# E3SM-Project/PAM

Measured on AMD Instinct MI355X. Metric: cell-updates/sec (AWFL dycore step), higher is better.
Workload: dtype f64; 1 GPU; AWFL supercell idealized, nens=1024/GPU, 32x32x60 L60, NT=1, fp64; scaling=weak, nens_total=1024, nens_per_gpu=1024, nx=32, ny=32, nz=60, num_tracers=1, parallelism=nens-shard x1, ranks_seen=1, limiter_input=0, fct_rows_flagged_last_stage=0, fct_rows=983040, lanes=member+xsweep

## Files before the change

### pam_amd/csrc/awfl_device.h

```cpp
#pragma once
#include <math.h>
#include <stdint.h>
#include <string.h>
#include <type_traits>
#include "awfl_constants.h"

#if defined(__HIPCC__)
#define PAMA_D __device__ __forceinline__
#else
#define PAMA_D inline
#endif

namespace pama {

constexpr int HS = 3;
constexpr int MAXT = 50;
constexpr int FLUX_THREADS = 256;
constexpr int FLUX_WAVES = FLUX_THREADS / 64;
#ifndef PAMA_FLUX_NF
#define PAMA_FLUX_NF 2
#endif
constexpr int FLUX_NF = PAMA_FLUX_NF;
constexpr int FLUX_MAX_SPAN = 64;
constexpr int VZ_STRIDE = 31;
// ... 1119 lines not shown
      const bool limited = (m != 1.0);
      if (limited) {
        rows.flags[(long long)t * fct_rows_per_tracer(P) + fct_row(P, k, j, i, e)] = rows.seq;
        rows.any[e >> 6] = rows.seq;
      }
      if (rows.sparse_store) store = wave_any(limited);
    }
    if (store) mult[(long long)t * P.ncell + idx] = m;
  }
}

PAMA_D double limited_flux(double F, double ml, double mh, bool seam) {
  if (F > 0.0) return mul_rn(F, ml);
  if (F < 0.0) return seam ? F : mul_rn(F, mh);
  return F;
}



struct NearFlags { bool c, im1, ip1, jm1, jp1, km1, kp1; };
PAMA_D bool any_of(const NearFlags &g) { return g.c | g.im1 | g.ip1 | g.jm1 | g.jp1 | g.km1 | g.kp1; }
PAMA_D NearFlags fct_near_flags(const Params &P, const FctRows &rows, int t, int k, int j, int i, int e) {
  const long long lstride = (long long)((P.nens + 63) >> 6) * P.nx;
  const int *fl = rows.flags + (long long)t * fct_rows_per_tracer(P) + fct_row(P, k, j, i, e);
  const long long r_ip1 = (i == P.nx - 1) ? -(long long)(P.nx - 1) : 1, r_im1 = (i == 0) ? (long long)(P.nx - 1) : -1;
  const long long r_jp1 = ((j == P.ny - 1) ? -(long long)(P.ny - 1) : 1) * lstride, r_jm1 = ((j == 0) ? (long long)(P.ny - 1) : -1) * lstride;
  const long long r_kz = (long long)P.ny * lstride;
  const bool zl = (k > 0), zh = (k < P.nz - 1);
  const int sq = rows.seq;
  const int a0 = fl[0], a1 = fl[r_im1], a2 = fl[r_ip1], a3 = fl[r_jm1], a4 = fl[r_jp1], a5 = fl[zl ? -r_kz : 0], a6 = fl[zh ? r_kz : 0];
  NearFlags g;
  g.c = (a0 == sq); g.im1 = (a1 == sq); g.ip1 = (a2 == sq); g.jm1 = (a3 == sq); g.jp1 = (a4 == sq);
  g.km1 = zl & (a5 == sq); g.kp1 = zh & (a6 == sq);
  return g;
}
PAMA_D bool fct_flagged_near(const Params &P, const FctRows &rows, int t, int k, int j, int i, int e) {
  return any_of(fct_near_flags(P, rows, t, k, j, i, e));
}

template <int STAGE>
PAMA_D void tracer_new_value(const Params &P, int t, double f_x, double f_xp1, double f_y, double f_yp1, double f_z, double f_zp1,
                             double q_in, double q_0, double rho_in, double rho_0, double rdzk, double dt_dyn, double &v,
                             double &new_seed) {
  const double tend = flux_divergence(P, f_x, f_xp1, f_y, f_yp1, f_z, f_zp1, rdzk);
  const double m_in = mul_rn(q_in, rho_in);
  double m_0 = 0.0;
  if (STAGE > 1) m_0 = mul_rn(q_0, rho_0);
  v = rk_combine<STAGE>(m_0, m_in, dt_dyn, tend);
  if ((P.pos_mask >> t) & 1ull) v = fmax(0.0, v);
  new_seed = next_seed<STAGE>(m_0, m_in, v);
}

template <int STAGE>
PAMA_D void tracer_update_one(const Params &P, int t, const double *prim_in, const double *prim0, double *prim_out,
                              const double *__restrict__ fx, const double *__restrict__ fy, const double *__restrict__ fz,
                              const double *__restrict__ mult, const FctRows &rows, double *__restrict__ seed, double dt_dyn,
                              const CellId &c, double rho_in, double rho_0, double rrho, double rdzk, bool only_near_flagged) {
  const int k = c.k, j = c.j, i = c.i, e = c.e;
  const long long idx = c.idx;
  const long long c2 = (long long)j * P.sy + (long long)i * P.sx + e;
  const long long o = (long long)(k + HS) * P.sz + c2;
  const long long ip1 = idx + ((i == P.nx - 1) ? -(long long)(P.nx - 1) * P.sx : P.sx);
  const long long im1 = idx + ((i == 0) ? (long long)(P.nx - 1) * P.sx : -P.sx);
  const long long jp1 = idx + ((j == P.ny - 1) ? -(long long)(P.ny - 1) * P.sy : P.sy);
  const long long jm1 = idx + ((j == 0) ? (long long)(P.ny - 1) * P.sy : -P.sy);
  const double *tx = fx + (long long)(5 + t) * P.ncell, *ty = fy + (long long)(5 + t) * P.ncell;
  const double *tz = fz + (long long)(5 + t) * P.fz_fs;
  const double *mt = mult + (long long)t * P.ncell;
  if (only_near_flagged && rows.flags) {
    if (!wave_any_or_lane(fct_flagged_near(P, rows, t, k, j, i, e))) return;
  }
  const bool zlo = (k > 0), zhi = (k < P.nz - 1);
  double m_c = 1.0, m_im1 = 1.0, m_ip1 = 1.0, m_jm1 = 1.0, m_jp1 = 1.0, m_km1 = 1.0, m_kp1 = 1.0;
  const double Fx = tx[idx], Fxp1 = tx[ip1], Fz = tz[idx], Fzp1 = tz[idx + P.sz];
  const double Fy = P.sim2d ? 0.0 : ty[idx], Fyp1 = P.sim2d ? 0.0 : ty[jp1];
  const int pf = P_TR0 + t;
  const double q_in = prim_in[pf * P.prim_fs + o];
  const double q_0 = (STAGE > 1) ? prim0[pf * P.prim_fs + o] : 0.0;
  if (rows.flags) {
    const NearFlags g = fct_near_flags(P, rows, t, k, j, i, e);
    if (wave_any(any_of(g))) {
      const double l_c = mt[idx], l_im1 = mt[im1], l_ip1 = mt[ip1], l_jm1 = mt[jm1], l_jp1 = mt[jp1];
      const double l_km1 = mt[zlo ? idx - P.sz : idx], l_kp1 = mt[zhi ? idx + P.sz : idx];
      m_c = g.c ? l_c : 1.0; m_im1 = g.im1 ? l_im1 : 1.0; m_ip1 = g.ip1 ? l_ip1 : 1.0;
      m_jm1 = g.jm1 ? l_jm1 : 1.0; m_jp1 = g.jp1 ? l_jp1 : 1.0;
      m_km1 = g.km1 ? l_km1 : 1.0; m_kp1 = g.kp1 ? l_kp1 : 1.0;
    }
  } else {
    m_c = mt[idx]; m_im1 = mt[im1]; m_ip1 = mt[ip1];
    if (!P.sim2d) { m_jm1 = mt[jm1]; m_jp1 = mt[jp1]; }
    if (zlo) m_km1 = mt[idx - P.sz];
    if (zhi) m_kp1 = mt[idx + P.sz];
  }
  double f_x = limited_flux(Fx, m_im1, m_c, i == 0);
  double f_xp1 = limited_flux(Fxp1, m_c, m_ip1, i == P.nx - 1);
  double f_y = 0.0, f_yp1 = 0.0;
  if (!P.sim2d) {
    f_y = limited_flux(Fy, m_jm1, m_c, j == 0);
    f_yp1 = limited_flux(Fyp1, m_c, m_jp1, j == P.ny - 1);
  }
  const double f_z = limited_flux(Fz, m_km1, m_c, false);
  const double f_zp1 = limited_flux(Fzp1, m_c, m_kp1, false);
  double v, new_seed;
  tracer_new_value<STAGE>(P, t, f_x, f_xp1, f_y, f_yp1, f_z, f_zp1, q_in, q_0, rho_in, rho_0, rdzk, dt_dyn, v, new_seed);
  seed[(long long)t * P.ncell + idx] = new_seed;
  store_adv(P, prim_out, pf, k, c2, v * rrho, v * rrho);
}

template <int STAGE>
PAMA_D void tracer_update_part(const Params &P, const double *prim_in, const double *prim0, double *prim_out,
                               const double *__restrict__ fx, const double *__restrict__ fy, const double *__restrict__ fz,
                               const double *__restrict__ mult, const FctRows &rows, double *__restrict__ seed, double dt_dyn,
                               const CellId &c, double rho_in, double rho_0, double rrho, double rdzk) {
  for (int t = 0; t < P.nt; t++)
    tracer_update_one<STAGE>(P, t, prim_in, prim0, prim_out, fx, fy, fz, mult, rows, seed, dt_dyn, c, rho_in, rho_0, rrho, rdzk, false);
}

template <int STAGE>
PAMA_D void tracer_fixup_line_body(const Params &P, const double *prim_in, const double *prim0, double *prim_out,
                                   const double *__restrict__ fx, const double *__restrict__ fy, const double *__restrict__ fz,
                                   const double *__restrict__ mult, const FctRows &rows, double *__restrict__ seed, double dt_dyn,
                                   int t, int k, int j, int e) {
  {
    const int *ln = rows.lines + (long long)t * fct_lines_per_tracer(P);
    const int sq = rows.seq;
    const bool zl = (k > 0), zh = (k < P.nz - 1);
    const int jm = (j == 0) ? P.ny - 1 : j - 1, jp = (j == P.ny - 1) ? 0 : j + 1;
    const int a0 = ln[fct_line(P, k, j, e)], a1 = ln[fct_line(P, k, jm, e)], a2 = ln[fct_line(P, k, jp, e)];
    const int a3 = ln[fct_line(P, zl ? k - 1 : k, j, e)], a4 = ln[fct_line(P, zh ? k + 1 : k, j, e)];
    if (!wave_any_or_lane((a0 == sq) | (a1 == sq) | (a2 == sq) | (a3 == sq) | (a4 == sq))) return;
  }
  const double rdzk = fast_rcp(P.dz[(long long)k * P.nens + e]);
  for (int i = 0; i < P.nx; i++) {
    if (!wave_any_or_lane(fct_flagged_near(P, rows, t, k, j, i, e))) continue;
    CellId c;
    c.k = k; c.j = j; c.i = i; c.e = e;
    c.idx = (((long long)k * P.ny + j) * P.nx + i) * P.nens + e;
    const long long o = (long long)(k + HS) * P.sz + (long long)j * P.sy + (long long)i * P.sx + e;
    const double rho_new = prim_out[P_RHO * P.prim_fs + o];
    const double rho_in = prim_in[P_RHO * P.prim_fs + o];
    const double rho_0 = (STAGE > 1) ? prim0[P_RHO * P.prim_fs + o] : 0.0;
    tracer_update_one<STAGE>(P, t, prim_in, prim0, prim_out, fx, fy, fz, mult, rows, seed, dt_dyn, c, rho_in, rho_0,
                             fast_rcp(rho_new), rdzk, false);
  }
}

template <int STAGE>
PAMA_D void tracer_fixup_cell_body(const Params &P, const double *prim_in, const double *prim0, double *prim_out,
                                   const double *__restrict__ fx, const double *__restrict__ fy, const double *__restrict__ fz,
                                   const double *__restrict__ mult, const FctRows &rows, double *__restrict__ seed, double dt_dyn,
                                   int t, const CellId &c) {
  const int k = c.k, j = c.j, e = c.e;
  {
    const int *ln = rows.lines + (long long)t * fct_lines_per_tracer(P);
    const int sq = rows.seq;
    const bool zl = (k > 0), zh = (k < P.nz - 1);
    const int jm = (j == 0) ? P.ny - 1 : j - 1, jp = (j == P.ny - 1) ? 0 : j + 1;
    const int a0 = ln[fct_line(P, k, j, e)], a1 = ln[fct_line(P, k, jm, e)], a2 = ln[fct_line(P, k, jp, e)];
    const int a3 = ln[fct_line(P, zl ? k - 1 : k, j, e)], a4 = ln[fct_line(P, zh ? k + 1 : k, j, e)];
    if (!wave_any_or_lane((a0 == sq) | (a1 == sq) | (a2 == sq) | (a3 == sq) | (a4 == sq))) return;
  }
  if (!wave_any_or_lane(fct_flagged_near(P, rows, t, k, j, c.i, e))) return;
  const double rdzk = fast_rcp(P.dz[(long long)k * P.nens + e]);
  const long long o = (long long)(k + HS) * P.sz + (long long)j * P.sy + (long long)c.i * P.sx + e;
  const double rho_new = prim_out[P_RHO * P.prim_fs + o];
  const double rho_in = prim_in[P_RHO * P.prim_fs + o];
  const double rho_0 = (STAGE > 1) ? prim0[P_RHO * P.prim_fs + o] : 0.0;
  tracer_update_one<STAGE>(P, t, prim_in, prim0, prim_out, fx, fy, fz, mult, rows, seed, dt_dyn, c, rho_in, rho_0,
                           fast_rcp(rho_new), rdzk, false);
}

PAMA_D void pressure_tail_body(const Params &P, double *prim_out, const CellId &c) {
  const long long c2 = (long long)c.j * P.sy + (long long)c.i * P.sx + c.e;
  const long long o = (long long)(c.k + HS) * P.sz + c2;
  const bool boundary = (c.k == 0 || c.k == P.nz - 1);
  const double th = boundary ? prim_out[P_THETA * P.prim_fs + o] : 0.0;
  const double rho_theta = prim_out[P_PRES * P.prim_fs + o];
  const double rho_new = boundary ? prim_out[P_RHO * P.prim_fs + o] : 0.0;
  store_rho_pres<false>(P, prim_out, c.k, c2, c.e, rho_new, th, rho_theta, !P.grav_balance);
}

template <int STAGE>
PAMA_D void update_body(const Params &P, const double *prim_in, const double *prim0,
                        double *prim_out, const double *__restrict__ fx, const double *__restrict__ fy,
                        const double *__restrict__ fz, const double *__restrict__ mult, const FctRows &rows,
                        double *__restrict__ seed, double dt_dyn, const CellId &c) {
  const int k = c.k, j = c.j, i = c.i, e = c.e;
  const long long idx = c.idx;
  const long long c2 = (long long)j * P.sy + (long long)i * P.sx + e;
  const long long o = (long long)(k + HS) * P.sz + c2;
  const long long ke = (long long)k * P.nens + e;
  const double dzk = P.dz[ke];
  const double rdzk = fast_rcp(dzk);
  const long long ip1 = idx + ((i == P.nx - 1) ? -(long long)(P.nx - 1) * P.sx : P.sx);
  const long long im1 = idx + ((i == 0) ? (long long)(P.nx - 1) * P.sx : -P.sx);
  const long long jp1 = idx + ((j == P.ny - 1) ? -(long long)(P.ny - 1) * P.sy : P.sy);
  const long long jm1 = idx + ((j == 0) ? (long long)(P.ny - 1) * P.sy : -P.sy);
  const double rho_in = prim_in[P_RHO * P.prim_fs + o];
  const double rho_0 = (STAGE > 1) ? prim0[P_RHO * P.prim_fs + o] : 0.0;
  double qs[5];
#pragma unroll
  for (int l = 0; l < 5; l++) {
    const double *sx_ = fx + (long long)l * P.ncell, *sy_ = fy + (long long)l * P.ncell, *sz_ = fz + (long long)l * P.fz_fs;
    const double ylo = P.sim2d ? 0.0 : sy_[idx], yhi = P.sim2d ? 0.0 : sy_[jp1];
    double tend = (l == 0) ? flux_divergence(P, sx_[idx], sx_[ip1], ylo, yhi, sz_[idx], sz_[idx + P.sz], rdzk)
                           : flux_divergence_d(P, sx_[idx], sx_[ip1], ylo - yhi, sz_[idx] - sz_[idx + P.sz], rdzk);
    if (l == 3) tend = add_gravity(P, tend, rho_in, gravity_coef(P, ke));
    if (l == 2 && P.sim2d) tend = 0.0;
    const int pf = (l == 0) ? P_RHO : P_U + (l - 1);
    double m_in = prim_in[pf * P.prim_fs + o];
    if (l > 0) m_in = mul_rn(m_in, rho_in);
    double m_0 = 0.0;
    if (STAGE > 1) {
      m_0 = prim0[pf * P.prim_fs + o];
      if (l > 0) m_0 = mul_rn(m_0, rho_0);
    }
    qs[l] = rk_combine<STAGE>(m_0, m_in, dt_dyn, tend);
  }
  const double rrho = fast_rcp(qs[0]);
  const double th = qs[4] * rrho;
  tracer_update_part<STAGE>(P, prim_in, prim0, prim_out, fx, fy, fz, mult, rows, seed, dt_dyn, c, rho_in, rho_0, rrho, rdzk);
  store_rho_pres(P, prim_out, k, c2, e, qs[0], th, qs[4], !P.grav_balance);
// ... 170 lines not shown
          }
          const double f_z = limited_flux(zl[n], m_km1[n], mB[n], false);
          const double f_zp1 = limited_flux(zh[n], mB[n], m_kp1[n], false);
          double v, new_seed;
          tracer_new_value<STAGE>(P, tt[n], f_x, f_xp1, f_y, f_yp1, f_z, f_zp1, w[n][1], q_0[n], rho_in, rho_0, rdzk, dt_dyn, v, new_seed);
          uniw(seed + (long long)tt[n] * P.ncell + ix)[eu] = new_seed;
          store_adv_u(P, prim_out, P_TR0 + tt[n], k, cu0 + (long long)cc * P.sx, eu, v * rrho, v * rrho);
        }
      }
      F_prev[n] = F;
      prevR[n] = R[n];
      mA[n] = mB[n];
      mB[n] = m_new[n];
#pragma unroll
      for (int s = 0; s < 4; s++) w[n][s] = w[n][s + 1];
      w[n][4] = nq[n];
    }
  }
}

template <int STAGE, bool FOLD = false>
PAMA_D void flux_x_update_body(const Params &P, const double *__restrict__ prim_in, const double *__restrict__ prim0,
                               double *__restrict__ prim_out, double *__restrict__ fx, const double *__restrict__ fy,
                               const double *__restrict__ fz, double *__restrict__ seed, double *__restrict__ mult,
                               const FctRows &rows, int line, int e, int c0, int span, double dt_dyn, double dt_stage,
                               bool tracers_inline) {
  const unsigned eu = member_offset(e);
  const WenoConsts wc = weno_consts();
  const int nx = P.nx;
  const int c1 = (c0 + span < nx) ? c0 + span : nx;
  const int k = uni_int(line / P.ny), j = line - k * P.ny;
  const long long cu0 = (long long)j * P.sy;
  const long long pbase = (long long)(k + HS) * P.sz + cu0;
  const long long fbase = (long long)k * P.sz + cu0;
  const long long jp1 = (j == P.ny - 1) ? -(long long)(P.ny - 1) * P.sy : P.sy;
  const long long ke = (long long)k * P.nens + e;
  const double dzk = P.dz[ke];
  const double rdzk = fast_rcp(dzk);
  const double gcoef = gravity_coef(P, ke);
  const bool have_y = !P.sim2d;
  double ruf_close = 0.0;
  double *ruf_line = fx + fbase;
  auto cell_off = [&](int c) -> long long { return pbase + (long long)(c < 0 ? c + nx : (c >= nx ? c - nx : c)) * P.sx; };

  {
    constexpr int NQ = 4;
    const double *pr = prim_in + (long long)P_RHO * P.prim_fs;
    const double *pp = prim_in + (long long)P_PRES * P.prim_fs;
    const double *r0 = prim0 + (long long)P_RHO * P.prim_fs;
    double *out_rho = prim_out + (long long)P_RHO * P.prim_fs, *out_rt = prim_out + (long long)P_PRES * P.prim_fs;
    double wm[5], wp[5], wq[NQ][5], wt[5];
    const int tr = P.idWV;
    const double *pt = prim_in + (long long)(P_TR0 + tr) * P.prim_fs;
    double *flt = fx + (long long)(5 + tr) * P.ncell + fbase;
    const bool more_tracers = P.nt > 1;
    auto load_cell = [&](long long o, double &m, double &p, double (&qv)[NQ]) {
#pragma unroll
      for (int n = 0; n < NQ; n++) qv[n] = uni(prim_in + (long long)(P_U + n) * P.prim_fs + o)[eu];
      m = mul_rn(uni(pr + o)[eu], qv[0]);
      p = uni(pp + o)[eu];
    };
#pragma unroll
    for (int s = 0; s < 5; s++) {
      double qv[NQ];
      load_cell(cell_off(c0 - 3 + s), wm[s], wp[s], qv);
#pragma unroll
      for (int n = 0; n < NQ; n++) wq[n][s] = qv[n];
      wt[s] = uni(pt + cell_off(c0 - 3 + s))[eu];
    }
    double prevR_m, prevR_p, prevR_q[NQ], prevR_t;
    {
      double L;
      weno5_const(wm, wc, L, prevR_m);
      weno5_const(wp, wc, L, prevR_p);
      weno5_const(wt, wc, L, prevR_t);
#pragma unroll
      for (int n = 0; n < NQ; n++) {
        if (n == 1 && !have_y) { prevR_q[n] = 0.0; continue; }
        weno5_const(wq[n], wc, L, prevR_q[n]);
      }
      double nm, np_, nq[NQ];
      load_cell(cell_off(c0 + 2), nm, np_, nq);
      const double nt0 = uni(pt + cell_off(c0 + 2))[eu];
#pragma unroll
      for (int s = 0; s < 4; s++) {
        wm[s] = wm[s + 1]; wp[s] = wp[s + 1]; wt[s] = wt[s + 1];
#pragma unroll
        for (int n = 0; n < NQ; n++) wq[n][s] = wq[n][s + 1];
      }
      wm[4] = nm; wp[4] = np_; wt[4] = nt0;
#pragma unroll
      for (int n = 0; n < NQ; n++) wq[n][4] = nq[n];
    }
    double F_prev[1 + NQ], Ft_prev = 0.0;
#pragma unroll
    for (int l = 0; l <= NQ; l++) F_prev[l] = 0.0;
    struct CellIn { double rho_in, rho_0, q0[NQ], y0l, y0h, z0l, z0h, dy[1 + NQ], dz[1 + NQ], tyl, tyh, tzl, tzh, tseed, tq0; };
    const double *fyt = fy + (long long)(5 + tr) * P.ncell, *fzt = fz + (long long)(5 + tr) * P.fz_fs;
    const double *pt0 = prim0 + (long long)(P_TR0 + tr) * P.prim_fs;
    const double *sdt = seed + (long long)tr * P.ncell;
    auto load_in = [&](int cc, CellIn &ci) {
      const long long o = pbase + (long long)cc * P.sx, ix = fbase + (long long)cc * P.sx;
      ci.rho_in = uni(pr + o)[eu];
      ci.rho_0 = (STAGE > 1) ? uni(r0 + o)[eu] : 0.0;
#pragma unroll
      for (int n = 0; n < NQ; n++) ci.q0[n] = (STAGE > 1) ? uni(prim0 + (long long)(P_U + n) * P.prim_fs + o)[eu] : 0.0;
      ci.y0l = have_y ? uni(fy + ix)[eu] : 0.0;
// ... 7 lines not shown
      }
      ci.tyl = have_y ? uni(fyt + ix)[eu] : 0.0;
      ci.tyh = have_y ? uni(fyt + ix + jp1)[eu] : 0.0;
      ci.tzl = uni(fzt + ix)[eu];
      ci.tzh = uni(fzt + ix + P.sz)[eu];
      ci.tseed = uni(sdt + ix)[eu];
      ci.tq0 = (STAGE > 1) ? uni(pt0 + o)[eu] : 0.0;
    };
    auto finish = [&](int cc, const CellIn &ci, const double (&Flo)[1 + NQ], const double (&Fhi)[1 + NQ], double m_in_u,
                      double v_in, double w_in, double th_in, double Ft_lo, double Ft_hi, double qt_in) {
      const long long o = pbase + (long long)cc * P.sx;
      const double q0 = rk_combine<STAGE>(ci.rho_0, ci.rho_in, dt_dyn,
                                          flux_divergence(P, Flo[0], Fhi[0], ci.y0l, ci.y0h, ci.z0l, ci.z0h, rdzk));
      const double rrho = fast_rcp(q0);
      uniw(out_rho + o)[eu] = q0;
      const double q_in[NQ] = {0.0, v_in, w_in, th_in};
#pragma unroll
      for (int n = 0; n < NQ; n++) {
        const int l = 1 + n;
        double tend = FOLD ? flux_divergence_g(P, Flo[l], Fhi[l], ci.dz[l]) : flux_divergence_d(P, Flo[l], Fhi[l], ci.dy[l], ci.dz[l], rdzk);
        if (l == 3) tend = add_gravity(P, tend, ci.rho_in, gcoef);
        if (l == 2 && P.sim2d) tend = 0.0;
        const double m_in = (n == 0) ? m_in_u : mul_rn(q_in[n], ci.rho_in);
        const double m_0 = (STAGE > 1) ? mul_rn(ci.q0[n], ci.rho_0) : 0.0;
        const double v = rk_combine<STAGE>(m_0, m_in, dt_dyn, tend);
        store_adv_u(P, prim_out, P_U + n, k, cu0 + (long long)cc * P.sx, eu, v * rrho, (l == 3) ? 0.0 : v * rrho);
        if (l == 4) uniw(out_rt + o)[eu] = v;
      }
      finish_tracer_cell<STAGE>(P, tr, prim_out, seed, mult, rows, k, j, cc, e, eu, cu0 + (long long)cc * P.sx, fbase + (long long)cc * P.sx,
                                Ft_lo, Ft_hi, ci.tyl, ci.tyh, ci.tzl, ci.tzh, ci.tseed, qt_in, ci.tq0, ci.rho_in, ci.rho_0, rrho, dzk,
                                rdzk, dt_dyn, dt_stage);
    };
#pragma clang loop unroll(disable)
    for (int c = c0; c <= c1; c++) {
      double nm, np_, nq[NQ];
      load_cell(cell_off(c + 3), nm, np_, nq);
      const double nt0 = uni(pt + cell_off(c + 3))[eu];
      CellIn ci;
      load_in(c > c0 ? c - 1 : c0, ci);
      double Lm, Rm, Lp, Rp, Lq[NQ], Rq[NQ];
      weno5_const(wm, wc, Lm, Rm);
      weno5_const(wp, wc, Lp, Rp);
#pragma unroll
      for (int n = 0; n < NQ; n++) {
        if (n == 1 && !have_y) { Lq[n] = Rq[n] = 0.0; continue; }
        weno5_const(wq[n], wc, Lq[n], Rq[n]);
      }
      double Lt, Rt;
      weno5_const(wt, wc, Lt, Rt);
      double ruf, ppf, F[1 + NQ];
      acoustic_face(prevR_m, Lm, prevR_p, Lp, false, ruf, ppf);
      const bool up = ruf > 0.0;
      const double Ft = mul_rn(ruf, up ? prevR_t : Lt);
      if (c < c1) {
        if (more_tracers) uniw(ruf_line + (long long)c * P.sx)[eu] = ruf;
        uniw(flt + (long long)c * P.sx)[eu] = Ft;
      }
      ruf_close = ruf;
      F[0] = ruf;
      F[1] = fma(ruf, up ? prevR_q[0] : Lq[0], ppf);
#pragma unroll
      for (int n = 1; n < NQ; n++) F[1 + n] = mul_rn(ruf, up ? prevR_q[n] : Lq[n]);
      if (c > c0) finish(c - 1, ci, F_prev, F, wm[1], wq[1][1], wq[2][1], wq[3][1], Ft_prev, Ft, wt[1]);
#pragma unroll
      for (int l = 0; l <= NQ; l++) F_prev[l] = F[l];
      Ft_prev = Ft;
      prevR_m = Rm; prevR_p = Rp; prevR_t = Rt;
#pragma unroll
      for (int n = 0; n < NQ; n++) prevR_q[n] = Rq[n];
#pragma unroll
      for (int s = 0; s < 4; s++) {
        wm[s] = wm[s + 1]; wp[s] = wp[s + 1]; wt[s] = wt[s + 1];
#pragma unroll
        for (int n = 0; n < NQ; n++) wq[n][s] = wq[n][s + 1];
      }
      wm[4] = nm; wp[4] = np_; wt[4] = nt0;
#pragma unroll
      for (int n = 0; n < NQ; n++) wq[n][4] = nq[n];
    }
  }

  if (tracers_inline) {
    for (int i = 0; i < P.nt - 1; i += FLUX_NF) {
      const int fa[2] = {4 + further_tracer(P, i), 4 + further_tracer(P, i + 1)};
      if (i + 1 < P.nt - 1) x_tracer_sweep<2, STAGE, 1>(P, prim_in, prim0, prim_out, fx, fy, fz, seed, mult, rows, line, e, c0, span, fa, dt_dyn, dt_stage, true, ruf_close);
      else x_tracer_sweep<1, STAGE, 1>(P, prim_in, prim0, prim_out, fx, fy, fz, seed, mult, rows, line, e, c0, span, fa, dt_dyn, dt_stage, true, ruf_close);
    }
  }
}

struct XTileGeom {
  int W;
  int nmb;
  int tc;
  int halo;
  int ntl;
  int lpb;
};
PAMA_HD int xtile_rows(const XTileGeom &G) { return G.tc + 2 * G.halo; }
PAMA_HD int xtile_threads(const XTileGeom &G) { return G.W * xtile_rows(G) * G.lpb; }
PAMA_HD XTileGeom xtile_geometry(const Params &P, int w_req, int tc_req, int lpb_req, int ncu = 0) {
  XTileGeom G;
  G.W = (P.nens <= 64) ? P.nens : 64;
  if (P.nens < 64 && (long long)P.nx * P.nens > 512) {
    const int nmb = (int)(((long long)P.nx * P.nens + 511) / 512), w = (P.nens + nmb - 1) / nmb;
    if (w >= 16 && P.nx * w <= 1024) G.W = w;
    else if ((long long)P.nx * P.nens > 1024) {
      const int nmb2 = (int)(((long long)P.nx * P.nens + 1023) / 1024), w2 = (P.nens + nmb2 - 1) / nmb2;
      if (w2 >= 16 && P.nx * w2 <= 1024) G.W = w2;
    }
// ... 783 lines not shown
```

### pam_amd/csrc/awfl_kernels.hip

```cpp
#include <hip/hip_runtime.h>

#include <cmath>
#include <cstdio>
#include <cstring>
#include <atomic>
#include <map>
#include <mutex>
#include <string>
#include <vector>

#include "../../include/pam_amd_awfl.h"
#include "awfl_device.h"
#include "awfl_vertical.h"

using namespace pama;

struct EnsRange { int e0, ne; };
__device__ __forceinline__ long long to_global(long long t, int nens, EnsRange R) {
  const long long r = t / R.ne;
  return r * nens + R.e0 + (t - r * R.ne);
}

__device__ __forceinline__ bool flat_cell(const Params &P, int nlev, CellId &c) {
  const unsigned t = blockIdx.x * blockDim.x + threadIdx.x;
// ... 240 lines not shown
  if (t >= (unsigned)P.nx * (unsigned)R.ne) return;
  CellId c;
  const unsigned i = t / (unsigned)R.ne;
  c.j = by; c.i = (int)i; c.e = R.e0 + (int)(t - i * (unsigned)R.ne);
#pragma unroll
  for (int kk = 0; kk < TAIL_LEVELS; kk++) {
    c.k = bz * TAIL_LEVELS + kk;
    if (c.k >= P.nz) return;
    c.idx = (((long long)c.k * P.ny + c.j) * P.nx + c.i) * P.nens + c.e;
    pressure_tail_body(P, prim_out, c);
  }
}
__global__ void __launch_bounds__(256) awfl_ptail_kernel(Params P, EnsRange R, double *__restrict__ prim_out) {
  __shared__ PowTab sh_tab;
  stage_pow_tab(P, &sh_tab);
  if (!P.flat_cells) { ptail_block(P, R, prim_out, blockIdx.x, (int)blockIdx.y, (int)blockIdx.z); return; }
  CellId c;
  const int ngrp = (P.nz + TAIL_LEVELS - 1) / TAIL_LEVELS;
  if (!flat_cell(P, ngrp, c)) return;
  const int kg = c.k;
#pragma unroll
  for (int kk = 0; kk < TAIL_LEVELS; kk++) {
    c.k = kg * TAIL_LEVELS + kk;
    if (c.k >= P.nz) return;
    c.idx = (((long long)c.k * P.ny + c.j) * P.nx + c.i) * P.nens + c.e;
    pressure_tail_body(P, prim_out, c);
  }
}
template <int STAGE>
__device__ __forceinline__ void trfix_block(const Params &P, EnsRange R, const double *__restrict__ prim_in,
                                            const double *__restrict__ prim0, double *prim_out,
                                            const double *__restrict__ fx, const double *__restrict__ fy,
                                            const double *__restrict__ fz, const double *__restrict__ mult,
                                            const FctRows &rows, double *__restrict__ seed, double dt_dyn, int block) {
  const int u = __builtin_amdgcn_readfirstlane((int)(block * 4 + (threadIdx.x >> 6)));
  const SweepUnits U = sweep_units(P.nz, P.ny, R.ne, 1, 1);
  const SweepUnits::Lane m = U.place(u);
  const int el = m.blk * 64 + (int)(threadIdx.x & 63);
  if (!U.holds(m, el)) return;
  if (rows.any[(R.e0 + el) >> 6] != rows.seq) return;
  const int k = uni_int(m.line / P.ny), j = m.line - k * P.ny;
  tracer_fixup_line_body<STAGE>(P, prim_in, prim0, prim_out, fx, fy, fz, mult, rows, seed, dt_dyn, P.idWV, k, j, R.e0 + el);
}
template <int STAGE>
__global__ void __launch_bounds__(256) awfl_trfix_kernel(Params P, EnsRange R, const double *__restrict__ prim_in,
                                                         const double *__restrict__ prim0, double *prim_out,
                                                         const double *__restrict__ fx, const double *__restrict__ fy,
                                                         const double *__restrict__ fz, const double *__restrict__ mult,
                                                         FctRows rows, double *__restrict__ seed, double dt_dyn) {
  fct_rows_resolve(rows);
  trfix_block<STAGE>(P, R, prim_in, prim0, prim_out, fx, fy, fz, mult, rows, seed, dt_dyn, (int)blockIdx.x);
}
template <int STAGE, bool SINGLES>
__global__ void __launch_bounds__(FLUX_THREADS) awfl_xtr2_tail_kernel(Params P, EnsRange R, const double *__restrict__ prim_in,
                                                                     const double *__restrict__ prim0, double *prim_out,
                                                                     const double *__restrict__ fx, const double *__restrict__ fy,
                                                                     const double *__restrict__ fz, double *__restrict__ seed,
                                                                     double *__restrict__ mult, FctRows rows, FctRows rows_fix, double dt_dyn,
                                                                     double dt_stage, int ngroups, int span, int nspan, int nb_xtr, int nb_pt,
                                                                     int ptx) {
  static_assert(FLUX_THREADS == 256, "the three bodies share workgroups of 256 lanes");
  __shared__ PowTab sh_tab;
  const int b = (int)blockIdx.x;
  if (b < nb_xtr) {
    fct_rows_resolve(rows);
    xtr_block<STAGE, 2, SINGLES ? 1 : 2>(P, R, prim_in, prim0, prim_out, fx, fy, fz, seed, mult, rows, dt_dyn, dt_stage, ngroups, span, nspan, b);
  } else if (b < nb_xtr + nb_pt) {
    stage_pow_tab(P, &sh_tab);
    const int q = b - nb_xtr, per_level = ptx * P.ny;
    const int bz = q / per_level, r = q - bz * per_level, by = r / ptx;
    ptail_block(P, R, prim_out, (unsigned)(r - by * ptx), by, bz);
  } else {
    fct_rows_resolve(rows_fix);
    trfix_block<STAGE>(P, R, prim_in, prim0, prim_out, fx, fy, fz, mult, rows_fix, seed, dt_dyn, b - nb_xtr - nb_pt);
  }
}
template <int STAGE>
__global__ void __launch_bounds__(256) awfl_trfix_flat_kernel(Params P, const double *__restrict__ prim_in,
                                                              const double *__restrict__ prim0, double *prim_out,
                                                              const double *__restrict__ fx, const double *__restrict__ fy,
                                                              const double *__restrict__ fz, const double *__restrict__ mult,
                                                              FctRows rows, double *__restrict__ seed, double dt_dyn) {
  fct_rows_resolve(rows);
  CellId c;
  if (!flat_cell(P, P.nz, c)) return;
  if (rows.any[c.e >> 6] != rows.seq) return;
  tracer_fixup_cell_body<STAGE>(P, prim_in, prim0, prim_out, fx, fy, fz, mult, rows, seed, dt_dyn, P.idWV, c);
}

template <bool SHUF>
struct XExchange {
  template <int N>
  static __device__ __forceinline__ void stage(const Params &P, const double *prim_in, const XLane &X, const int (&fields)[N], double *st,
                                               int TS, double (&own)[N], unsigned fmask = ~0u) {
    if (SHUF) {
      xtile_load_own<N>(P, prim_in, X, fields, own, fmask);
    } else {
      xtile_stage<N>(P, prim_in, X, fields, st, TS, own, fmask);
      __syncthreads();
    }
  }
  template <int N>
  static __device__ __forceinline__ double nb(const XLane &X, const XShuf &S, const double *st, int TS, const double (&own)[N], int f, int s) {
    return SHUF ? xtile_shfl(own[f], S.ln[s]) : st[f * TS + X.s5[s]];
  }
};
template <int STAGE, int PHASE, int NF, bool SHUF>
// ... 159 lines not shown
  fct_rows_resolve(rows);
  extern __shared__ double xt_lds[];
  const int T = (int)(blockDim.x * blockDim.y * blockDim.z);
  const int tid = (int)((threadIdx.z * blockDim.y + threadIdx.y) * blockDim.x + threadIdx.x);
  const XLane X = xtile_lane(P, G, (int)blockIdx.x, (int)blockIdx.y, (int)threadIdx.x, (int)threadIdx.y, (int)threadIdx.z);
  const int TS = xtile_stage_elems(G);
  XShuf S = {};
  if (SHUF) S = xtile_shuffle_lanes(P, G, tid & 63, (int)threadIdx.x, (int)threadIdx.y);
  const int nz_state = state_parts ? 3 : 1;
  if ((int)blockIdx.z >= nz_state) {
    const int i = 2 * ((int)blockIdx.z - nz_state);
    const int fa[2] = {4 + further_tracer(P, i), 4 + further_tracer(P, i + 1)};
    if (i + 1 < P.nt - 1)
      xtr_tile_run_own_flux<STAGE, 2, SHUF>(P, X, S, T, TS, prim_in, prim0, prim_out, fx, fy, fz, seed, mult, rows, dt_dyn, dt_stage, fa, xt_lds);
    else
      xtr_tile_run_own_flux<STAGE, 1, SHUF>(P, X, S, T, TS, prim_in, prim0, prim_out, fx, fy, fz, seed, mult, rows, dt_dyn, dt_stage, fa, xt_lds);
    return;
  }
  double F[XT_NF];
  if (state_parts) {
    if (blockIdx.z == 0) xupd_tile_state<STAGE, SHUF, XP_U>(P, X, S, T, TS, prim_in, prim0, prim_out, fx, fy, fz, seed, mult, rows, dt_dyn, dt_stage, with_pressure != 0, xt_lds, F);
    else if (blockIdx.z == 1) xupd_tile_state<STAGE, SHUF, XP_VW>(P, X, S, T, TS, prim_in, prim0, prim_out, fx, fy, fz, seed, mult, rows, dt_dyn, dt_stage, with_pressure != 0, xt_lds, F);
    else xupd_tile_state<STAGE, SHUF, XP_T>(P, X, S, T, TS, prim_in, prim0, prim_out, fx, fy, fz, seed, mult, rows, dt_dyn, dt_stage, with_pressure != 0, xt_lds, F);
    return;
  }
  xupd_tile_state<STAGE, SHUF, XP_ALL>(P, X, S, T, TS, prim_in, prim0, prim_out, fx, fy, fz, seed, mult, rows, dt_dyn, dt_stage, with_pressure != 0, xt_lds, F);
  if (tracers_inline == 1) {
    for (int i = 0; i < P.nt - 1; i += 2) {
      const int fa[2] = {4 + further_tracer(P, i), 4 + further_tracer(P, i + 1)};
      if (!SHUF) __syncthreads();
      if (i + 1 < P.nt - 1)
        xtr_tile_run<STAGE, 1, 2, SHUF>(P, X, S, T, TS, prim_in, prim0, prim_out, fx, fy, fz, seed, mult, rows, dt_dyn, dt_stage, fa, xt_lds, true, F[0]);
      else
        xtr_tile_run<STAGE, 1, 1, SHUF>(P, X, S, T, TS, prim_in, prim0, prim_out, fx, fy, fz, seed, mult, rows, dt_dyn, dt_stage, fa, xt_lds, true, F[0]);
    }
  }
}
template <int STAGE, int PHASE, bool SHUF>
__global__ void __launch_bounds__(1024) awfl_xtr_tile_kernel(Params P, XTileGeom G, const double *__restrict__ prim_in,
                                                             const double *__restrict__ prim0, double *__restrict__ prim_out,
                                                             const double *__restrict__ fx, const double *__restrict__ fy,
                                                             const double *__restrict__ fz, double *__restrict__ seed,
                                                             double *__restrict__ mult, FctRows rows, double dt_dyn,
                                                             double dt_stage, int fixup_slice) {
  fct_rows_resolve(rows);
  extern __shared__ double xt_lds[];
  const int pair = (int)blockIdx.z;
  const int T = (int)(blockDim.x * blockDim.y * blockDim.z);
  const XLane X = xtile_lane(P, G, (int)blockIdx.x, (int)blockIdx.y, (int)threadIdx.x, (int)threadIdx.y, (int)threadIdx.z);
  if (PHASE == 2 && fixup_slice && pair == (int)gridDim.z - 1) {
    if (X.upd && rows.any[X.e >> 6] == rows.seq) {
      CellId c;
      c.k = X.k; c.j = X.j; c.i = X.i; c.e = X.e; c.idx = (long long)X.io;
      tracer_fixup_cell_body<STAGE>(P, prim_in, prim0, prim_out, fx, fy, fz, mult, rows, seed, dt_dyn, P.idWV, c);
    }
    return;
  }
  const int TS = xtile_stage_elems(G);
  XShuf S = {};
  if (SHUF) S = xtile_shuffle_lanes(P, G, (int)((threadIdx.z * blockDim.y + threadIdx.y) * blockDim.x + threadIdx.x) & 63, (int)threadIdx.x, (int)threadIdx.y);
  const int fa[2] = {4 + further_tracer(P, 2 * pair), 4 + further_tracer(P, 2 * pair + 1)};
  if (2 * pair + 1 < P.nt - 1)
    xtr_tile_run<STAGE, PHASE, 2, SHUF>(P, X, S, T, TS, prim_in, prim0, prim_out, fx, fy, fz, seed, mult, rows, dt_dyn, dt_stage, fa, xt_lds, false, 0.0);
  else
    xtr_tile_run<STAGE, PHASE, 1, SHUF>(P, X, S, T, TS, prim_in, prim0, prim_out, fx, fy, fz, seed, mult, rows, dt_dyn, dt_stage, fa, xt_lds, false, 0.0);
}

constexpr int FT_MAXG = (4 + MAXT + FT_NG - 1) / FT_NG + 1;
struct FTileGroups { int ny_groups, nz_groups; int gy[FT_MAXG][FT_NG], gz[FT_MAXG][FT_NG]; };
template <int DIR>
__device__ __forceinline__ void ftile_workgroup_lane(const Params &P, const FTileGeom &G, int bx, int by, FLane &X) {
  const int rows = ftile_rows(G), per = rows * G.W;
  const int t = (int)threadIdx.x;
  const int tz = t / per, r = t - tz * per, ty = r / G.W, tx = r - ty * G.W;
  X = ftile_lane<DIR>(P, G, bx, by, tx, ty, tz < G.lpb ? tz : 0);
  if (tz >= G.lpb) { X.poly = X.face = X.own = X.pay = false; X.slot = X.slot_l = X.slot_r = 0; }
}
template <int DIR, bool VZ_PER_ENS>
__device__ __forceinline__ void flux_tile_run(const Params &P, const FTileGeom &G, int bx, int by, int T, const int (*grp)[FT_NG],
                                              int ngroups, const double *__restrict__ prim, double *__restrict__ flux, double *lds) {
  FLane X;
  ftile_workgroup_lane<DIR>(P, G, bx, by, X);
  double *ldsR[2] = {lds, lds + FT_NG * T}, *ldsF = lds + 2 * FT_NG * T;
  const int ncomp_a = (DIR == 1) ? 1 : 2;
  double L[FT_NG], R[FT_NG], F[FT_NG], ruf = 0.0, fn = 0.0;
  if (X.poly) {
    ftile_acoustic_polys<DIR, VZ_PER_ENS>(P, prim, X, L, R);
#pragma unroll
    for (int n = 0; n < FT_NG; n++) ldsR[0][n * T + X.slot] = R[n];
  }
  __syncthreads();
  if (X.face) {
#pragma unroll
    for (int n = 0; n < FT_NG; n++) R[n] = ldsR[0][n * T + X.slot_l];
    ftile_acoustic_face<DIR>(P, flux, X, L, R, ruf, fn);
    ldsF[X.slot] = fn;
  }
  for (int g = 0; g < ngroups; g++) {
    double *buf = ldsR[(g + 1) & 1];
    int fa[FT_NG], nf = 0;
#pragma unroll
    for (int n = 0; n < FT_NG; n++) { fa[n] = grp[g][n]; nf += (fa[n] >= 0) ? 1 : 0; }
    if (X.poly) {
      ftile_adv_polys<DIR, VZ_PER_ENS>(P, prim, X, fa, nf, L, R);
#pragma unroll
      for (int n = 0; n < FT_NG; n++) buf[n * T + X.slot] = R[n];
    }
// ... 1938 lines not shown
```

Measured before the change: 2.728 billion cell-updates/s.

## Recompute water-vapor x-face fluxes in FCT fixup instead of storing them

Stops the x-sweep from writing the per-cell limited-tracer x flux for the water-vapor tracer to global memory. The line and cell fixup paths now recompute those faces from the input primitives with WENO5 and the acoustic Riemann face. This removes a full-field store from the hot sweep at the cost of extra recomputation on flagged fixup rows, which are reported as zero here. Launch bounds on the xtr2 tail kernel are also given a minimum occupancy hint, which may force register spills.

Result: no change. 2.758 billion cell-updates/s (median of 6 runs) (+1.1%).

```diff
diff --git a/pam_amd/csrc/awfl_device.h b/pam_amd/csrc/awfl_device.h
--- a/pam_amd/csrc/awfl_device.h
+++ b/pam_amd/csrc/awfl_device.h
@@ -1195,10 +1195,10 @@
 }
 
 template <int STAGE>
-PAMA_D void tracer_update_one(const Params &P, int t, const double *prim_in, const double *prim0, double *prim_out,
-                              const double *__restrict__ fx, const double *__restrict__ fy, const double *__restrict__ fz,
-                              const double *__restrict__ mult, const FctRows &rows, double *__restrict__ seed, double dt_dyn,
-                              const CellId &c, double rho_in, double rho_0, double rrho, double rdzk, bool only_near_flagged) {
+PAMA_D void tracer_update_faces(const Params &P, int t, const double *prim_in, const double *prim0, double *prim_out, double Fx,
+                                double Fxp1, const double *__restrict__ fy, const double *__restrict__ fz,
+                                const double *__restrict__ mult, const FctRows &rows, double *__restrict__ seed, double dt_dyn,
+                                const CellId &c, double rho_in, double rho_0, double rrho, double rdzk) {
   const int k = c.k, j = c.j, i = c.i, e = c.e;
   const long long idx = c.idx;
   const long long c2 = (long long)j * P.sy + (long long)i * P.sx + e;
@@ -1207,15 +1207,12 @@
   const long long im1 = idx + ((i == 0) ? (long long)(P.nx - 1) * P.sx : -P.sx);
   const long long jp1 = idx + ((j == P.ny - 1) ? -(long long)(P.ny - 1) * P.sy : P.sy);
   const long long jm1 = idx + ((j == 0) ? (long long)(P.ny - 1) * P.sy : -P.sy);
-  const double *tx = fx + (long long)(5 + t) * P.ncell, *ty = fy + (long long)(5 + t) * P.ncell;
+  const double *ty = fy + (long long)(5 + t) * P.ncell;
   const double *tz = fz + (long long)(5 + t) * P.fz_fs;
   const double *mt = mult + (long long)t * P.ncell;
-  if (only_near_flagged && rows.flags) {
-    if (!wave_any_or_lane(fct_flagged_near(P, rows, t, k, j, i, e))) return;
-  }
   const bool zlo = (k > 0), zhi = (k < P.nz - 1);
   double m_c = 1.0, m_im1 = 1.0, m_ip1 = 1.0, m_jm1 = 1.0, m_jp1 = 1.0, m_km1 = 1.0, m_kp1 = 1.0;
-  const double Fx = tx[idx], Fxp1 = tx[ip1], Fz = tz[idx], Fzp1 = tz[idx + P.sz];
+  const double Fz = tz[idx], Fzp1 = tz[idx + P.sz];
   const double Fy = P.sim2d ? 0.0 : ty[idx], Fyp1 = P.sim2d ? 0.0 : ty[jp1];
   const int pf = P_TR0 + t;
   const double q_in = prim_in[pf * P.prim_fs + o];
@@ -1248,6 +1245,20 @@
   tracer_new_value<STAGE>(P, t, f_x, f_xp1, f_y, f_yp1, f_z, f_zp1, q_in, q_0, rho_in, rho_0, rdzk, dt_dyn, v, new_seed);
   seed[(long long)t * P.ncell + idx] = new_seed;
   store_adv(P, prim_out, pf, k, c2, v * rrho, v * rrho);
+}
+template <int STAGE>
+PAMA_D void tracer_update_one(const Params &P, int t, const double *prim_in, const double *prim0, double *prim_out,
+                              const double *__restrict__ fx, const double *__restrict__ fy, const double *__restrict__ fz,
+                              const double *__restrict__ mult, const FctRows &rows, double *__restrict__ seed, double dt_dyn,
+                              const CellId &c, double rho_in, double rho_0, double rrho, double rdzk, bool only_near_flagged) {
+  const long long idx = c.idx;
+  const long long ip1 = idx + ((c.i == P.nx - 1) ? -(long long)(P.nx - 1) * P.sx : P.sx);
+  const double *tx = fx + (long long)(5 + t) * P.ncell;
+  if (only_near_flagged && rows.flags) {
+    if (!wave_any_or_lane(fct_flagged_near(P, rows, t, c.k, c.j, c.i, c.e))) return;
+  }
+  tracer_update_faces<STAGE>(P, t, prim_in, prim0, prim_out, tx[idx], tx[ip1], fy, fz, mult, rows, seed, dt_dyn, c, rho_in, rho_0, rrho,
+                             rdzk);
 }
 
 template <int STAGE>
@@ -1273,26 +1284,100 @@
     const int a3 = ln[fct_line(P, zl ? k - 1 : k, j, e)], a4 = ln[fct_line(P, zh ? k + 1 : k, j, e)];
     if (!wave_any_or_lane((a0 == sq) | (a1 == sq) | (a2 == sq) | (a3 == sq) | (a4 == sq))) return;
   }
+  (void)fx;
   const double rdzk = fast_rcp(P.dz[(long long)k * P.nens + e]);
-  for (int i = 0; i < P.nx; i++) {
-    if (!wave_any_or_lane(fct_flagged_near(P, rows, t, k, j, i, e))) continue;
-    CellId c;
-    c.k = k; c.j = j; c.i = i; c.e = e;
-    c.idx = (((long long)k * P.ny + j) * P.nx + i) * P.nens + e;
-    const long long o = (long long)(k + HS) * P.sz + (long long)j * P.sy + (long long)i * P.sx + e;
-    const double rho_new = prim_out[P_RHO * P.prim_fs + o];
-    const double rho_in = prim_in[P_RHO * P.prim_fs + o];
-    const double rho_0 = (STAGE > 1) ? prim0[P_RHO * P.prim_fs + o] : 0.0;
-    tracer_update_one<STAGE>(P, t, prim_in, prim0, prim_out, fx, fy, fz, mult, rows, seed, dt_dyn, c, rho_in, rho_0,
-                             fast_rcp(rho_new), rdzk, false);
-  }
-}
-
-template <int STAGE>
-PAMA_D void tracer_fixup_cell_body(const Params &P, const double *prim_in, const double *prim0, double *prim_out,
-                                   const double *__restrict__ fx, const double *__restrict__ fy, const double *__restrict__ fz,
-                                   const double *__restrict__ mult, const FctRows &rows, double *__restrict__ seed, double dt_dyn,
-                                   int t, const CellId &c) {
+  const unsigned eu = member_offset(e);
+  const WenoConsts wc = weno_consts();
+  const int nx = P.nx;
+  const long long pbase = (long long)(k + HS) * P.sz + (long long)j * P.sy;
+  const double *pr = prim_in + (long long)P_RHO * P.prim_fs, *pu = prim_in + (long long)P_U * P.prim_fs;
+  const double *pp = prim_in + (long long)P_PRES * P.prim_fs, *pt = prim_in + (long long)(P_TR0 + t) * P.prim_fs;
+  auto load_cell = [&](int c, double &m, double &p, double &q) {
+    const long long o = pbase + (long long)(c < 0 ? c + nx : (c >= nx ? c - nx : c)) * P.sx;
+    m = mul_rn(uni(pr + o)[eu], uni(pu + o)[eu]);
+    p = uni(pp + o)[eu];
+    q = uni(pt + o)[eu];
+  };
+  double wm[5], wp[5], wt[5];
+#pragma unroll
+  for (int s = 0; s < 5; s++) load_cell(s - 3, wm[s], wp[s], wt[s]);
+  double prevR_m, prevR_p, prevR_t;
+  {
+    double L;
+    weno5_const(wm, wc, L, prevR_m);
+    weno5_const(wp, wc, L, prevR_p);
+    weno5_const(wt, wc, L, prevR_t);
+    double nm, np_, nt0;
+    load_cell(2, nm, np_, nt0);
+#pragma unroll
+    for (int s = 0; s < 4; s++) { wm[s] = wm[s + 1]; wp[s] = wp[s + 1]; wt[s] = wt[s + 1]; }
+    wm[4] = nm; wp[4] = np_; wt[4] = nt0;
+  }
+  double Ft_prev = 0.0;
+#pragma clang loop unroll(disable)
+  for (int c = 0; c <= nx; c++) {
+    double nm, np_, nt0;
+    load_cell(c + 3, nm, np_, nt0);
+    double Lm, Rm, Lp, Rp, Lt, Rt;
+    weno5_const(wm, wc, Lm, Rm);
+    weno5_const(wp, wc, Lp, Rp);
+    weno5_const(wt, wc, Lt, Rt);
+    double ruf, ppf;
+    acoustic_face(prevR_m, Lm, prevR_p, Lp, false, ruf, ppf);
+    const bool up = ruf > 0.0;
+    const double Ft = mul_rn(ruf, up ? prevR_t : Lt);
+    const int i = c - 1;
+    if (c > 0 && wave_any_or_lane(fct_flagged_near(P, rows, t, k, j, i, e))) {
+      CellId cl;
+      cl.k = k; cl.j = j; cl.i = i; cl.e = e;
+      cl.idx = (((long long)k * P.ny + j) * P.nx + i) * P.nens + e;
+      const long long o = pbase + (long long)i * P.sx + e;
+      const double rho_new = prim_out[P_RHO * P.prim_fs + o];
+      const double rho_in = prim_in[P_RHO * P.prim_fs + o];
+      const double rho_0 = (STAGE > 1) ? prim0[P_RHO * P.prim_fs + o] : 0.0;
+      tracer_update_faces<STAGE>(P, t, prim_in, prim0, prim_out, Ft_prev, Ft, fy, fz, mult, rows, seed, dt_dyn, cl, rho_in, rho_0,
+                                 fast_rcp(rho_new), rdzk);
+    }
+    Ft_prev = Ft;
+    prevR_m = Rm; prevR_p = Rp; prevR_t = Rt;
+#pragma unroll
+    for (int s = 0; s < 4; s++) { wm[s] = wm[s + 1]; wp[s] = wp[s + 1]; wt[s] = wt[s + 1]; }
+    wm[4] = nm; wp[4] = np_; wt[4] = nt0;
+  }
+}
+
+PAMA_D double tracer_x_face_from_input(const Params &P, const double *prim_in, int t, int k, int j, int f, int e) {
+  const WenoConsts wc = weno_consts();
+  const int nx = P.nx;
+  const long long base = (long long)(k + HS) * P.sz + (long long)j * P.sy + e;
+  const double *pr = prim_in + (long long)P_RHO * P.prim_fs, *pu = prim_in + (long long)P_U * P.prim_fs;
+  const double *pp = prim_in + (long long)P_PRES * P.prim_fs, *pt = prim_in + (long long)(P_TR0 + t) * P.prim_fs;
+  double wm[6], wp[6], wt[6];
+#pragma unroll
+  for (int s = 0; s < 6; s++) {
+    const int c = f - 3 + s;
+    const long long o = base + (long long)(c < 0 ? c + nx : (c >= nx ? c - nx : c)) * P.sx;
+    wm[s] = mul_rn(pr[o], pu[o]);
+    wp[s] = pp[o];
+    wt[s] = pt[o];
+  }
+  double L, R, prevR_m, prevR_p, prevR_t, Lm, Lp, Lt;
+  weno5_const(wm, wc, L, prevR_m);
+  weno5_const(wp, wc, L, prevR_p);
+  weno5_const(wt, wc, L, prevR_t);
+  weno5_const(wm + 1, wc, Lm, R);
+  weno5_const(wp + 1, wc, Lp, R);
+  weno5_const(wt + 1, wc, Lt, R);
+  double ruf, ppf;
+  acoustic_face(prevR_m, Lm, prevR_p, Lp, false, ruf, ppf);
+  return mul_rn(ruf, (ruf > 0.0) ? prevR_t : Lt);
+}
+
+template <int STAGE, bool STORED_X>
+PAMA_D void tracer_fixup_cell(const Params &P, const double *prim_in, const double *prim0, double *prim_out,
+                              const double *__restrict__ fx, const double *__restrict__ fy, const double *__restrict__ fz,
+                              const double *__restrict__ mult, const FctRows &rows, double *__restrict__ seed, double dt_dyn, int t,
+                              const CellId &c) {
   const int k = c.k, j = c.j, e = c.e;
   {
     const int *ln = rows.lines + (long long)t * fct_lines_per_tracer(P);
@@ -1309,8 +1394,23 @@
   const double rho_new = prim_out[P_RHO * P.prim_fs + o];
   const double rho_in = prim_in[P_RHO * P.prim_fs + o];
   const double rho_0 = (STAGE > 1) ? prim0[P_RHO * P.prim_fs + o] : 0.0;
-  tracer_update_one<STAGE>(P, t, prim_in, prim0, prim_out, fx, fy, fz, mult, rows, seed, dt_dyn, c, rho_in, rho_0,
-                           fast_rcp(rho_new), rdzk, false);
+  if (STORED_X) {
+    tracer_update_one<STAGE>(P, t, prim_in, prim0, prim_out, fx, fy, fz, mult, rows, seed, dt_dyn, c, rho_in, rho_0,
+                             fast_rcp(rho_new), rdzk, false);
+    return;
+  }
+  double F[2];
+#pragma clang loop unroll(disable)
+  for (int s = 0; s < 2; s++) F[s] = tracer_x_face_from_input(P, prim_in, t, k, j, c.i + s, e);
+  tracer_update_faces<STAGE>(P, t, prim_in, prim0, prim_out, F[0], F[1], fy, fz, mult, rows, seed, dt_dyn, c, rho_in, rho_0,
+                             fast_rcp(rho_new), rdzk);
+}
+template <int STAGE>
+PAMA_D void tracer_fixup_cell_body(const Params &P, const double *prim_in, const double *prim0, double *prim_out,
+                                   const double *__restrict__ fx, const double *__restrict__ fy, const double *__restrict__ fz,
+                                   const double *__restrict__ mult, const FctRows &rows, double *__restrict__ seed, double dt_dyn,
+                                   int t, const CellId &c) {
+  tracer_fixup_cell<STAGE, false>(P, prim_in, prim0, prim_out, fx, fy, fz, mult, rows, seed, dt_dyn, t, c);
 }
 
 PAMA_D void pressure_tail_body(const Params &P, double *prim_out, const CellId &c) {
@@ -1587,7 +1687,6 @@
     double wm[5], wp[5], wq[NQ][5], wt[5];
     const int tr = P.idWV;
     const double *pt = prim_in + (long long)(P_TR0 + tr) * P.prim_fs;
-    double *flt = fx + (long long)(5 + tr) * P.ncell + fbase;
     const bool more_tracers = P.nt > 1;
     auto load_cell = [&](long long o, double &m, double &p, double (&qv)[NQ]) {
 #pragma unroll
@@ -1701,10 +1800,7 @@
       acoustic_face(prevR_m, Lm, prevR_p, Lp, false, ruf, ppf);
       const bool up = ruf > 0.0;
       const double Ft = mul_rn(ruf, up ? prevR_t : Lt);
-      if (c < c1) {
-        if (more_tracers) uniw(ruf_line + (long long)c * P.sx)[eu] = ruf;
-        uniw(flt + (long long)c * P.sx)[eu] = Ft;
-      }
+      if (c < c1 && more_tracers) uniw(ruf_line + (long long)c * P.sx)[eu] = ruf;
       ruf_close = ruf;
       F[0] = ruf;
       F[1] = fma(ruf, up ? prevR_q[0] : Lq[0], ppf);
diff --git a/pam_amd/csrc/awfl_kernels.hip b/pam_amd/csrc/awfl_kernels.hip
--- a/pam_amd/csrc/awfl_kernels.hip
+++ b/pam_amd/csrc/awfl_kernels.hip
@@ -316,7 +316,7 @@
   trfix_block<STAGE>(P, R, prim_in, prim0, prim_out, fx, fy, fz, mult, rows, seed, dt_dyn, (int)blockIdx.x);
 }
 template <int STAGE, bool SINGLES>
-__global__ void __launch_bounds__(FLUX_THREADS) awfl_xtr2_tail_kernel(Params P, EnsRange R, const double *__restrict__ prim_in,
+__global__ void __launch_bounds__(FLUX_THREADS, SINGLES ? 4 : 3) awfl_xtr2_tail_kernel(Params P, EnsRange R, const double *__restrict__ prim_in,
                                                                      const double *__restrict__ prim0, double *prim_out,
                                                                      const double *__restrict__ fx, const double *__restrict__ fy,
                                                                      const double *__restrict__ fz, double *__restrict__ seed,
@@ -582,7 +582,7 @@
     if (X.upd && rows.any[X.e >> 6] == rows.seq) {
       CellId c;
       c.k = X.k; c.j = X.j; c.i = X.i; c.e = X.e; c.idx = (long long)X.io;
-      tracer_fixup_cell_body<STAGE>(P, prim_in, prim0, prim_out, fx, fy, fz, mult, rows, seed, dt_dyn, P.idWV, c);
+      tracer_fixup_cell<STAGE, true>(P, prim_in, prim0, prim_out, fx, fy, fz, mult, rows, seed, dt_dyn, P.idWV, c);
     }
     return;
   }
```
